# dgaddy/silent_speech

Hardware: AMD Instinct MI355X
Metric: EMG frames/s training (transduction_model.py) (higher is better)
Workload: dtype bf16

## Files before the change

include/silent_speech_hip.h:

```cpp
#ifndef SILENT_SPEECH_HIP_H
#define SILENT_SPEECH_HIP_H
#include <stdint.h>
#ifdef __cplusplus
extern "C" {
#endif

#define SS_F32 0
#define SS_BF16 1
#define SS_F32X3 3

const char* ss_last_error(void);
#define SS_ABI_VERSION 23
int ss_abi_version(void);
const char* ss_target_arch(void);

typedef struct ss_rowmap {
    int64_t base;
    int64_t batch_stride;
    int64_t row_stride;
    int32_t rows_per_batch;
} ss_rowmap;

typedef struct ss_gemm_epilogue {
    const float* bias;
    const void* gate;
    float gate_scale;
    float alpha;
// ... 114 lines not shown

int ss_emg_prepare(int dtype, const float* x_raw, void* out_padded, float* shifted_copy, int B, int T0, int Cin, int shift, void* stream);

int ss_loss_index_tables(const int64_t* utt_dev, int n_utt, int32_t* vo_pred, int32_t* vo_tgt, int32_t* si_tgt, int32_t* si_base,
                         int32_t* si_res, void* stream);
int ss_frame_lse(const float* head, int64_t ld, int col0, int ncls, int rows, float* lse, int32_t* argmax, void* stream);
int ss_voiced_loss(const float* head, int64_t ld, int n_mel, int n_phone, const float* lse, const int32_t* argmax, const float* Y,
                   const int64_t* phones, const int32_t* pred_row, const int32_t* tgt_row, int nframes, float lam, float inv_total,
                   float* dhead, float* loss_accum, int32_t* correct_accum, void* stream);
int ss_silent_cost_skewed(const float* head, int64_t ld, int n_mel, const float* lse, const float* Y, const int64_t* phones,
                          const int64_t* desc_dev, int n, int max_n, int max_m, float lam, void* workspace, int32_t* results, void* stream);
int ss_silent_loss(const float* head, int64_t ld, int n_mel, int n_phone, const float* lse, const int32_t* argmax, const float* Y,
                   const int64_t* phones, const int32_t* results, const int32_t* tgt_row, const int32_t* pred_base,
                   const int32_t* res_idx, int nframes, float lam, float inv_total, float* dhead, float* loss_accum,
                   int32_t* correct_accum, void* stream);
int ss_phoneme_confusion(const int32_t* argmax, const int64_t* phones, const int32_t* results, const int32_t* vo_pred, const int32_t* vo_tgt,
                         int n_voiced, const int32_t* si_tgt, const int32_t* si_base, const int32_t* si_res, int n_silent_frames,
                         int32_t* confusion, int n_phone, void* stream);

int ss_ctc_loss(const float* logits, int64_t ld, int V, int blank, const float* lse, const int64_t* desc_dev, int n_utt, int max_target_len,
                int64_t rows, const int32_t* targets, float* alpha_ws, float* beta_ws, float* nll, float* dlogits, float* loss, void* stream);

int64_t ss_ctc_beam_workspace_bytes(int n_utt, int64_t total_frames, int beam_width);
int ss_ctc_beam_search(const float* logits, int64_t ld, int V, int blank, int64_t rows, const float* lse, const int64_t* utt_dev, int n_utt,
                       int64_t total_frames, int beam_width, int n_best, const float* lm, float alpha, float beta, void* workspace, int max_len,
                       int32_t* labels, int32_t* lengths, float* scores, float* ctc_scores, void* stream);

typedef struct ss_word_lm {
    const int32_t* lex_child;
    const int32_t* lex_word;
// ... 184 lines not shown
```

silent_speech_amd/_lib.py:

```python
import ctypes
import os

import torch

_HERE = os.path.dirname(os.path.abspath(__file__))
_LIB_PATH = os.environ.get('SS_AMD_LIBRARY') or os.path.join(_HERE, 'lib', 'libsilent_speech_hip.so')

SS_F32, SS_BF16, SS_F64, SS_F32X3 = 0, 1, 2, 3
ABI_VERSION = 23
OP_KC, OP_OC = 0, 1


class RowMap(ctypes.Structure):
    _fields_ = [('base', ctypes.c_int64), ('batch_stride', ctypes.c_int64), ('row_stride', ctypes.c_int64),
                ('rows_per_batch', ctypes.c_int32)]


class GemmEpilogue(ctypes.Structure):
    _fields_ = [('bias', ctypes.c_void_p), ('gate', ctypes.c_void_p), ('gate_scale', ctypes.c_float),
                ('alpha', ctypes.c_float), ('relu', ctypes.c_int32), ('dropout_p', ctypes.c_float),
                ('seed', ctypes.c_uint64), ('rng_stream', ctypes.c_uint32), ('mode', ctypes.c_int32),
                ('col_mod', ctypes.c_int32), ('col_mul', ctypes.c_int32), ('col_div_mul', ctypes.c_int32),
                ('log_clamp', ctypes.c_float), ('c2', ctypes.c_void_p), ('cmap2', RowMap), ('col_stride2', ctypes.c_int64),
                ('col_sum', ctypes.c_void_p), ('col_sumsq', ctypes.c_void_p), ('col_shift', ctypes.c_void_p),
# ... 22 lines not shown
    _fields_ = [('lex_child', ctypes.c_void_p), ('lex_word', ctypes.c_void_p), ('uni_logp', ctypes.c_void_p), ('uni_bo', ctypes.c_void_p),
                ('bi_keys', ctypes.c_void_p), ('bi_logp', ctypes.c_void_p), ('bi_bo', ctypes.c_void_p), ('tri_keys', ctypes.c_void_p),
                ('tri_logp', ctypes.c_void_p), ('n_nodes', ctypes.c_int32), ('n_vocab', ctypes.c_int32), ('n_uni', ctypes.c_int32),
                ('start', ctypes.c_int32), ('bi_slots', ctypes.c_int32), ('bi_probe', ctypes.c_int32), ('tri_slots', ctypes.c_int32),
                ('tri_probe', ctypes.c_int32)]


class WordStateLm(ctypes.Structure):
    _fields_ = [('lex_child', ctypes.c_void_p), ('lex_word', ctypes.c_void_p), ('uni_logp', ctypes.c_void_p), ('st_bo', ctypes.c_void_p),
                ('st_shorter', ctypes.c_void_p), ('arc_keys', ctypes.c_void_p), ('arc_logp', ctypes.c_void_p), ('arc_next', ctypes.c_void_p),
                ('n_nodes', ctypes.c_int32), ('n_vocab', ctypes.c_int32), ('n_uni', ctypes.c_int32), ('n_states', ctypes.c_int32),
                ('start_state', ctypes.c_int32), ('arc_slots', ctypes.c_int32), ('arc_probe', ctypes.c_int32), ('order', ctypes.c_int32)]


_P, _I, _F, _L = ctypes.c_void_p, ctypes.c_int, ctypes.c_float, ctypes.c_int64
_U64, _U32 = ctypes.c_uint64, ctypes.c_uint32

SIGNATURES = {
    'ss_gemm': [_I, _I, _I, _I, _P, _P, _P, _I, _I, _I, ctypes.POINTER(RowMap), ctypes.POINTER(RowMap),
                ctypes.POINTER(RowMap), ctypes.POINTER(GemmEpilogue), _I, _P],
    'ss_gemm_dw_grouped': [_I, ctypes.POINTER(DwJob), _P],
    'ss_split_planes': [_P, _P, _P, _L, _P],
    'ss_gemm_planes': [_I, _P, _P, _P, _P, _P, _I, _I, _I, ctypes.POINTER(RowMap), ctypes.POINTER(RowMap), ctypes.POINTER(RowMap), ctypes.POINTER(GemmEpilogue), _P],
    'ss_permute3d': [_P, _I, _P, _I, _I, _I, _I, _L, _L, _L, _I, _I, _F, _I, _P],
    'ss_permute3d_batch': [_P, _P, _I, _I, _P],
    'ss_dtw_align': [_P, _P, _I, _I, _I, _P, _P, _P],
    'ss_dtw_align_skewed': [_P, _I, _P, _P, _P],
    'ss_reflect_pad_ragged': [_P, _P, _P, _P, _I, _I, _I, _L, _I, _P],
    'ss_concat_pad': [_P, _I, _P, _L, _I, _P],
    'ss_dtw_cumulative': [_I, _P, _L, _L, _I, _I, _P, _P, _P],
# ... 14 lines not shown
    'ss_bn_backward_sums': [_I, _P, _I, _P, _I, _P, _I, _P, _P, _P, _I, _P, _P, _P, _P, _P, _P, _P, _P, _I, _I, _I, _I, _P, _P, _P, _P, _P],
    'ss_bn_backward_apply': [_I, _P, _I, _P, _I, _P, _I, _P, _P, _P, _P, _I, _P, _P, _P, _P, ctypes.c_double, _P, _I, _P, _I, _I, _I, _I, _I, _P, _P, _P],
    'ss_colsum': [_I, _P, _I, _I, _L, _P, _P, _P],
    'ss_add_dropout_layernorm_forward': [_I, _P, _P, _P, _P, _P, _P, _P, _I, _I, _F, _F, _U64, _U32, _P],
    'ss_add_dropout_layernorm_forward_planes': [_I, _P, _P, _P, _P, _P, _P, _P, _P, _P, _I, _I, _F, _F, _U64, _U32, _P],
    'ss_layernorm_backward': [_I, _P, _P, _P, _P, _P, _P, _P, _P, _P, _I, _I, _F, _U64, _U32, _P],
    'ss_layernorm_backward_bias': [_I, _P, _P, _P, _P, _P, _P, _P, _P, _P, _P, _I, _I, _F, _U64, _U32, _P],
    'ss_layernorm_backward_ws': [_I, _P, _P, _P, _P, _P, _P, _P, _P, _P, _P, _P, _L, _I, _I, _F, _U64, _U32, _P],
    'ss_layernorm_backward_ws_planes': [_I, _P, _P, _P, _P, _P, _P, _P, _P, _P, _P, _P, _P, _P, _L, _I, _I, _F, _U64, _U32, _P],
    'ss_emg_prepare': [_I, _P, _P, _P, _I, _I, _I, _I, _P],
    'ss_frame_lse': [_P, _L, _I, _I, _I, _P, _P, _P],
    'ss_loss_index_tables': [_P, _I, _P, _P, _P, _P, _P, _P],
    'ss_voiced_loss': [_P, _L, _I, _I, _P, _P, _P, _P, _P, _P, _I, _F, _F, _P, _P, _P, _P],
    'ss_silent_cost_skewed': [_P, _L, _I, _P, _P, _P, _P, _I, _I, _I, _F, _P, _P, _P],
    'ss_silent_loss': [_P, _L, _I, _I, _P, _P, _P, _P, _P, _P, _P, _P, _I, _F, _F, _P, _P, _P, _P],
    'ss_phoneme_confusion': [_P, _P, _P, _P, _P, _I, _P, _P, _P, _I, _P, _I, _P],
    'ss_ctc_loss': [_P, _L, _I, _I, _P, _P, _I, _I, _L, _P, _P, _P, _P, _P, _P, _P],
    'ss_ctc_beam_search': [_P, _L, _I, _I, _L, _P, _P, _I, _L, _I, _I, _P, _F, _F, _P, _I, _P, _P, _P, _P, _P],
    'ss_ctc_word_beam_search': [_P, _L, _I, _I, _I, _L, _P, _P, _I, _L, _I, _I, ctypes.POINTER(WordLm), _F, _F, _P, _I, _P, _P, _P, _P, _P, _P],
    'ss_word_ngram_score': [ctypes.POINTER(WordLm), _P, _L, _P, _P],
    'ss_ctc_word_state_beam_search': [_P, _L, _I, _I, _I, _L, _P, _P, _I, _L, _I, _I, ctypes.POINTER(WordStateLm), _F, _F, _P, _I, _P, _P, _P, _P, _P, _P],
    'ss_word_state_score': [ctypes.POINTER(WordStateLm), _P, _L, _P, _P, _P],
    'ss_ctc_align': [_P, _L, _I, _I, _L, _P, _P, _I, _L, _I, _P, _L, _P, _P, _P, _P, _P, _P, _P],
    'ss_edit_distance': [_P, _L, _P, _L, _P, _L, _P, _P, _P, _P, _L, _P, _P],
    'ss_nbest_risk': [_P, _L, _P, _L, _P, _I, _I, _P, _P, _L, _P, _P, _P],
    'ss_ctc_nbest_logp': [_P, _L, _I, _I, _L, _P, _P, _I, _P, _L, _I, _P, _L, _P, _L, _P, _P],
    'ss_ctc_nbest_backward': [_P, _L, _I, _I, _L, _P, _P, _I, _L, _P, _P, _L, _P, _P, _P, _P],
    'ss_nbest_expected_risk': [_P, _P, _L, _P, _I, ctypes.c_double, _P, _P, _P, _P, _P],
    'ss_adamw_step': [_P, _P, _P, _P, _L, _F, _F, _F, _F, _F, _I, _F, _P],
    'ss_cast_f32': [_P, _P, _I, _L, _P],
# ... 162 lines not shown
```

silent_speech_amd/csrc/loss.hip:

```cpp
#include "common.h"
#include <stdlib.h>
#include "silent_speech_hip.h"
#include <math.h>

namespace {
constexpr int DESC = 10;
enum { D_N = 0, D_M, D_PRED_ROW0, D_TGT_ROW0, D_UNUSED, D_SK_OFF, D_DIRS_OFF, D_BND_OFF, D_RES_OFF };
constexpr int DW = 4, DR = 4;
__device__ __forceinline__ long long dtw_strips_d(long long n) { long long rows = n - 1, cap = DW * 64 * DR; return rows <= 0 ? 0 : (rows + cap - 1) / cap; }
__device__ __forceinline__ long long dtw_tsteps_d(long long m) { return m <= 1 ? 0 : (m - 1) + 63; }
}

__global__ void frame_lse_kernel(const float* __restrict__ head, long long ld, int col0, int ncls, int rows, float* __restrict__ lse, int* __restrict__ amax)
{
    const int lane = threadIdx.x & 63, wpb = blockDim.x >> 6;
    for (int r = blockIdx.x * wpb + (threadIdx.x >> 6); r < rows; r += gridDim.x * wpb) {
        const float* a = head + (long long)r * ld + col0;
        float mx = -INFINITY; int mi = 0x7fffffff;
        for (int c = lane; c < ncls; c += 64) { float v = a[c]; if (v > mx) { mx = v; mi = c; } }
        const float gmx = wave_max(mx);
        int cand = (mx == gmx) ? mi : 0x7fffffff;
#pragma unroll
        for (int m = 32; m >= 1; m >>= 1) { int o = __shfl_xor(cand, m); cand = o < cand ? o : cand; }
        float s = 0.f;
// ... 44 lines not shown
__device__ __forceinline__ void loss_block_commit(float lsum, int csum, float inv_total, float* loss_acc, int* correct_acc)
{
    __shared__ float ls[16];
    __shared__ int cs[16];
    const int lane = threadIdx.x & 63, w = threadIdx.x >> 6, wpb = blockDim.x >> 6;
    if (lane == 0) { ls[w] = lsum; cs[w] = csum; }
    __syncthreads();
    if (threadIdx.x == 0) {
        float a = 0.f; int c = 0;
        for (int i = 0; i < wpb; ++i) { a += ls[i]; c += cs[i]; }
        if (a != 0.f) atomicAdd(loss_acc, a * inv_total);
        if (c) atomicAdd(correct_acc, c);
    }
}

__global__ void voiced_loss_kernel(const float* __restrict__ head, long long ld, int n_mel, int n_ph, const float* __restrict__ lse, const int* __restrict__ amax,
                                   const float* __restrict__ Y, const long long* __restrict__ phones, const int* __restrict__ pred_row, const int* __restrict__ tgt_row,
                                   int nframes, float lam, float inv_total, float* __restrict__ dhead, float* __restrict__ loss_acc, int* __restrict__ correct_acc)
{
    const int lane = threadIdx.x & 63, wpb = blockDim.x >> 6;
    float lsum = 0.f; int csum = 0;
    for (int f = blockIdx.x * wpb + (threadIdx.x >> 6); f < nframes; f += gridDim.x * wpb) {
        const int pr = pred_row[f], tr = tgt_row[f];
        const float* p = head + (long long)pr * ld; const float* y = Y + (long long)tr * n_mel;
        float* dp = dhead + (long long)pr * ld;
        float ss = 0.f;
        for (int c = lane; c < n_mel; c += 64) { float d = y[c] - p[c] + 1e-6f; ss += d * d; }
        const float dist = sqrtf(wave_sum(ss));
        const float gs = dist > 0.f ? inv_total / dist : 0.f;
        for (int c = lane; c < n_mel; c += 64) dp[c] = -(y[c] - p[c] + 1e-6f) * gs;
        const int ph = (int)phones[tr];
        const float L = lse[pr];
        for (int c = lane; c < n_ph; c += 64) dp[n_mel + c] = lam * inv_total * (expf(p[n_mel + c] - L) - (c == ph ? 1.f : 0.f));
        if (lane == 0) { lsum += dist + lam * (L - p[n_mel + ph]); csum += amax[pr] == ph; }
    }
    loss_block_commit(lsum, csum, inv_total, loss_acc, correct_acc);
}

extern "C" int ss_voiced_loss(const float* head, int64_t ld, int n_mel, int n_phone, const float* lse, const int32_t* argmax, const float* Y, const int64_t* phones,
                              const int32_t* pred_row, const int32_t* tgt_row, int nframes, float lam, float inv_total,
                              float* dhead, float* loss_accum, int32_t* correct_accum, void* stream)
{
    SS_CHECK(nframes >= 0, "ss_voiced_loss: negative frame count");
    if (nframes == 0) return 0;
    SS_CHECK(head && lse && argmax && Y && phones && pred_row && tgt_row && dhead && loss_accum && correct_accum, "ss_voiced_loss: null pointer");
    int blocks = (nframes + 3) / 4; if (blocks > 1024) blocks = 1024;
    SS_LAUNCH(voiced_loss_kernel, dim3(blocks), dim3(256), 0, stream, head, (long long)ld, n_mel, n_phone, lse, (const int*)argmax, Y, (const long long*)phones,
              (const int*)pred_row, (const int*)tgt_row, nframes, lam, inv_total, dhead, loss_accum, (int*)correct_accum);
    SS_LAUNCH_CHECK("ss_voiced_loss");
    return 0;
}

constexpr int YMAX = 128;
__device__ __forceinline__ float quad_bcast(float v, int k) {
#if defined(SS_EMU)
    return __shfl(v, (int)((threadIdx.x & 63) & ~3) + k);
#else
    switch (k) {
    case 0: return __int_as_float(__builtin_amdgcn_update_dpp(0, __float_as_int(v), 0x00, 0xf, 0xf, true));
    case 1: return __int_as_float(__builtin_amdgcn_update_dpp(0, __float_as_int(v), 0x55, 0xf, 0xf, true));
    case 2: return __int_as_float(__builtin_amdgcn_update_dpp(0, __float_as_int(v), 0xAA, 0xf, 0xf, true));
    default: return __int_as_float(__builtin_amdgcn_update_dpp(0, __float_as_int(v), 0xFF, 0xf, 0xf, true));
    }
#endif
}
template <int NQ>
__device__ __forceinline__ float quad_shared_sqdist(const float* __restrict__ p, int r, const f32x4 (&yv)[YMAX / 4]) {
    f32x4 own[NQ];
#pragma unroll
    for (int q = 0; q < NQ; ++q) own[q] = *(const f32x4*)(p + (r * NQ + q) * 4);
    float ss = 0.f;
#pragma unroll
    for (int k = 0; k < 4; ++k) {
#pragma unroll
        for (int q = 0; q < NQ; ++q) {
            const f32x4 b = yv[k * NQ + q];
            const float a0 = quad_bcast(own[q][0], k), a1 = quad_bcast(own[q][1], k), a2 = quad_bcast(own[q][2], k), a3 = quad_bcast(own[q][3], k);
            const float d0 = a0 - b[0], d1 = a1 - b[1], d2 = a2 - b[2], d3 = a3 - b[3];
            ss += d0 * d0; ss += d1 * d1; ss += d2 * d2; ss += d3 * d3;
        }
    }
    return ss;
}

__global__ __launch_bounds__(256) void silent_cost_skewed_kernel(const float* __restrict__ head, long long ld, int n_mel, const float* __restrict__ lse, const float* __restrict__ Y,
                                                                 const long long* __restrict__ phones, const long long* __restrict__ desc, float lam, unsigned char* __restrict__ ws, int* __restrict__ results, int CT)
{
    const long long* d = desc + (long long)blockIdx.y * DESC;
    const int N = (int)d[D_N], M = (int)d[D_M];
    const long long p0 = d[D_PRED_ROW0], y0 = d[D_TGT_ROW0];
    int* res = results + d[D_RES_OFF];
    for (int i = blockIdx.x * blockDim.x + threadIdx.x; i < N; i += gridDim.x * blockDim.x) res[i] = 0;
    const long long ts = dtw_tsteps_d(M), nkw = dtw_strips_d(N) * DW;
    if (ts <= 0) return;
    const long long tchunks = (ts + CT - 1) / CT, nwork = nkw * tchunks;
    float* sk = (float*)(ws + d[D_SK_OFF]);
    const int l = threadIdx.x >> 2, r = threadIdx.x & 3;
    for (long long wk = blockIdx.x; wk < nwork; wk += gridDim.x) {
        const long long kw = wk / tchunks, t0 = (wk - kw * tchunks) * CT;
        const long long i = 1 + (kw * 64 + l) * DR + r;
        const bool iv = i < N;
        f32x4 yv[YMAX / 4];
        int ph = 0;
        if (iv) {
            const float* y = Y + (y0 + i) * n_mel;
#pragma unroll
            for (int q = 0; q < YMAX / 4; ++q) if (q * 4 < n_mel) yv[q] = *(const f32x4*)(y + q * 4);
            ph = (int)phones[y0 + i];
        }
        const long long tend = t0 + CT < ts ? t0 + CT : ts;
        if (n_mel == 80) {
            for (long long t = t0; t < tend; ++t) {
                const long long j = t + 1 - l;
                const bool jv = j >= 1 && j < M;
                const float* p = head + (p0 + (jv ? j : 1)) * ld;
                const float ss = quad_shared_sqdist<5>(p, r, yv);
                float c = INFINITY;
                if (jv && iv) c = sqrtf(ss) + lam * (lse[p0 + j] - p[n_mel + ph]);
                sk[((kw * ts + t) * 64 + l) * DR + r] = c;
            }
            continue;
        }
        for (long long t = t0; t < tend; ++t) {
            const long long j = t + 1 - l;
            float c = INFINITY;
            if (iv && j >= 1 && j < M) {
                const float* p = head + (p0 + j) * ld;
// ... 11 lines not shown
            sk[((kw * ts + t) * 64 + l) * DR + r] = c;
        }
    }
}

extern "C" int ss_silent_cost_skewed(const float* head, int64_t ld, int n_mel, const float* lse, const float* Y, const int64_t* phones,
                                     const int64_t* desc_dev, int n, int max_n, int max_m, float lam, void* workspace, int32_t* results, void* stream)
{
    SS_CHECK(n >= 0, "ss_silent_cost_skewed: negative batch");
    if (n == 0) return 0;
    SS_CHECK(head && lse && Y && phones && desc_dev && workspace && results, "ss_silent_cost_skewed: null pointer");
    SS_CHECK(n_mel % 4 == 0 && ld % 4 == 0, "ss_silent_cost_skewed: n_mel and ld must be multiples of 4 (16-byte rows)");
    SS_CHECK(n_mel <= YMAX, "ss_silent_cost_skewed: at most %d mel bins", YMAX);
    long long strips = max_n <= 1 ? 0 : (max_n - 1 + DW * 64 * DR - 1) / (DW * 64 * DR);
    const long long ts_max = max_m <= 1 ? 0 : max_m - 1 + 63;
    static const int CT = getenv("SS_COST_CT") ? atoi(getenv("SS_COST_CT")) : 16;
    long long blocks = strips * DW * ((ts_max + CT - 1) / CT);
    if (blocks < (max_n + 255) / 256) blocks = (max_n + 255) / 256;
    if (blocks > 4096) blocks = 4096;
    if (blocks < 1) blocks = 1;
    SS_LAUNCH(silent_cost_skewed_kernel, dim3((unsigned)blocks, n), dim3(256), 0, stream, head, (long long)ld, n_mel, lse, Y, (const long long*)phones,
              (const long long*)desc_dev, lam, (unsigned char*)workspace, (int*)results, CT);
    SS_LAUNCH_CHECK("ss_silent_cost_skewed");
    return 0;
}

__global__ void silent_loss_kernel(const float* __restrict__ head, long long ld, int n_mel, int n_ph, const float* __restrict__ lse, const int* __restrict__ amax,
                                   const float* __restrict__ Y, const long long* __restrict__ phones, const int* __restrict__ results,
                                   const int* __restrict__ tgt_row, const int* __restrict__ pred_base, const int* __restrict__ res_idx,
                                   int nframes, float lam, float inv_total, float* __restrict__ dhead, float* __restrict__ loss_acc, int* __restrict__ correct_acc)
{
    const int lane = threadIdx.x & 63, wpb = blockDim.x >> 6;
    float lsum = 0.f; int csum = 0;
    for (int f = blockIdx.x * wpb + (threadIdx.x >> 6); f < nframes; f += gridDim.x * wpb) {
        const int tr = tgt_row[f], pr = pred_base[f] + results[res_idx[f]];
        const float* p = head + (long long)pr * ld; const float* y = Y + (long long)tr * n_mel;
        float* dp = dhead + (long long)pr * ld;
        float ss = 0.f;
        for (int c = lane; c < n_mel; c += 64) { float d = p[c] - y[c]; ss += d * d; }
        const float dist = sqrtf(wave_sum(ss));
        const float gs = dist > 0.f ? inv_total / dist : 0.f;
        for (int c = lane; c < n_mel; c += 64) atomicAdd(dp + c, (p[c] - y[c]) * gs);
        const int ph = (int)phones[tr];
        const float L = lse[pr];
        for (int c = lane; c < n_ph; c += 64) atomicAdd(dp + n_mel + c, lam * inv_total * (expf(p[n_mel + c] - L) - (c == ph ? 1.f : 0.f)));
        if (lane == 0) { lsum += dist + lam * (L - p[n_mel + ph]); csum += amax[pr] == ph; }
    }
    loss_block_commit(lsum, csum, inv_total, loss_acc, correct_acc);
}

extern "C" int ss_silent_loss(const float* head, int64_t ld, int n_mel, int n_phone, const float* lse, const int32_t* argmax, const float* Y, const int64_t* phones,
                              const int32_t* results, const int32_t* tgt_row, const int32_t* pred_base, const int32_t* res_idx, int nframes,
                              float lam, float inv_total, float* dhead, float* loss_accum, int32_t* correct_accum, void* stream)
{
    SS_CHECK(nframes >= 0, "ss_silent_loss: negative frame count");
    if (nframes == 0) return 0;
    SS_CHECK(head && lse && argmax && Y && phones && results && tgt_row && pred_base && res_idx && dhead && loss_accum && correct_accum, "ss_silent_loss: null pointer");
    int blocks = (nframes + 3) / 4; if (blocks > 1024) blocks = 1024;
    SS_LAUNCH(silent_loss_kernel, dim3(blocks), dim3(256), 0, stream, head, (long long)ld, n_mel, n_phone, lse, (const int*)argmax, Y, (const long long*)phones,
              (const int*)results, (const int*)tgt_row, (const int*)pred_base, (const int*)res_idx, nframes, lam, inv_total, dhead, loss_accum, (int*)correct_accum);
    SS_LAUNCH_CHECK("ss_silent_loss");
    return 0;
}

__global__ void phoneme_confusion_kernel(const int* __restrict__ amax, const long long* __restrict__ phones, const int* __restrict__ results,
                                         const int* __restrict__ vo_pred, const int* __restrict__ vo_tgt, int n_voiced,
                                         const int* __restrict__ si_tgt, const int* __restrict__ si_base, const int* __restrict__ si_res, int n_silent,
                                         int* __restrict__ conf, int n_phone)
{
    for (int i = blockIdx.x * blockDim.x + threadIdx.x; i < n_voiced + n_silent; i += gridDim.x * blockDim.x) {
        int p, t;
        if (i < n_voiced) { p = amax[vo_pred[i]]; t = (int)phones[vo_tgt[i]]; }
        else { const int k = i - n_voiced; p = amax[si_base[k] + results[si_res[k]]]; t = (int)phones[si_tgt[k]]; }
        if ((unsigned)p < (unsigned)n_phone && (unsigned)t < (unsigned)n_phone) atomicAdd(conf + p * n_phone + t, 1);
        else atomicAdd(conf + n_phone * n_phone, 1);
    }
// ... 18 lines not shown
```

silent_speech_amd/ops.py:

```python
import ctypes

import torch

from . import _lib
from ._lib import OP_KC, OP_OC, RowMap, GemmEpilogue


def rowmap(row_stride, rows_per_batch=0, batch_stride=0, base=0):
    return RowMap(int(base), int(batch_stride), int(row_stride), int(rows_per_batch))


PROFILER = None


class LaunchProfiler(object):

    def __init__(self):
        self.records = []
        self.enabled = True

    def run(self, name, flops, nbytes, fn):
        if not self.enabled or not torch.cuda.is_available():
            return fn()
        s = torch.cuda.Event(enable_timing=True)
# ... 9 lines not shown
        agg = {}
        for name, flops, nbytes, s, e in self.records:
            a = agg.setdefault(name, dict(calls=0, flops=0.0, bytes=0.0, seconds=0.0))
            a['calls'] += 1
            a['flops'] += flops
            a['bytes'] += nbytes
            a['seconds'] += s.elapsed_time(e) * 1e-3
        self.records = []
        return agg


def timed(name, flops, nbytes, fn):
    if PROFILER is not None:
        return PROFILER.run(name, flops, nbytes, fn)
    return fn()


def gemm(A, B, C, M, N, K, amap, bmap, cmap, **kw):
    return _gemm_full(A, B, C, M, N, K, amap, bmap, cmap, {}, **kw)


def permute3d(inp, out, dims, strides, valid1=None, valid2=None, scale=1.0, accumulate=False):
    d0, d1, d2 = dims
    assert out.numel() >= d0 * d1 * d2 and out.is_contiguous()
    rc = _lib.lib().ss_permute3d(_lib.ptr(inp), _lib.dtype_code(inp.dtype), _lib.ptr(out), _lib.dtype_code(out.dtype),
                                 d0, d1, d2, strides[0], strides[1], strides[2],
                                 d1 if valid1 is None else valid1, d2 if valid2 is None else valid2,
                                 float(scale), int(accumulate), _lib.stream_of(out))
    _lib.check(rc, 'ss_permute3d')
    return out
# ... 438 lines not shown
```

silent_speech_amd/torch_ops.py:

```python
import ctypes
import weakref
from typing import Optional, Tuple

import torch
from torch import Tensor

from . import _lib, ops

_L = _lib.lib
_p = _lib.ptr

_models = {}
_next_id = [1]
_KEEP = 2


def model_handle(model):
    h = getattr(model, '_op_handle', None)
    if h is None:
        h = model._op_handle = _next_id[0]
        _next_id[0] += 1
        _models[h] = weakref.ref(model)
        model._saved_ctx = {}
    return h
# ... 66 lines not shown


@model_forward_ragged.register_fake
def _(x_raw, lens, handle):
    m = _model(handle)
    n_head_cols = (m.num_outs + (m.num_aux_outs or 0) + 7) // 8 * 8
    return x_raw.new_empty((x_raw.shape[0] * (x_raw.shape[1] // 8), n_head_cols), dtype=torch.float32)


@torch.library.custom_op('silent_speech::dtw_loss', mutates_args=())
def dtw_loss(head: Tensor, Y: Tensor, phones: Tensor, idx: Tensor, desc: Tensor, n_mel: int, n_ph: int, lam: float, inv_total: float,
             n_voiced: int, n_silent_frames: int, n_silent: int, ws_bytes: int, res_total: int, max_n: int, max_m: int,
             cells: float, perimeter: float) -> Tuple[Tensor, Tensor, Tensor, Tensor, Tensor]:
    dev = head.device
    M, ld = head.shape
    st = _lib.stream_of(head)
    nv, ns = max(n_voiced, 1), max(n_silent_frames, 1)
    vo_pred, vo_tgt = idx[:nv], idx[nv:2 * nv]
    si_tgt, si_base, si_res = idx[2 * nv:2 * nv + ns], idx[2 * nv + ns:2 * nv + 2 * ns], idx[2 * nv + 2 * ns:]
    lse = torch.empty(M, dtype=torch.float32, device=dev)
    amax = torch.empty(M, dtype=torch.int32, device=dev)
    dhead = torch.zeros_like(head)
    loss = torch.zeros(1, dtype=torch.float32, device=dev)
    correct = torch.zeros(1, dtype=torch.int32, device=dev)
    _lib.check(_L().ss_frame_lse(_p(head), ld, n_mel, n_ph, M, _p(lse), _p(amax), st), 'ss_frame_lse')
    if n_voiced:
        _lib.check(_L().ss_voiced_loss(_p(head), ld, n_mel, n_ph, _p(lse), _p(amax), _p(Y), _p(phones), _p(vo_pred), _p(vo_tgt),
                                       n_voiced, lam, inv_total, _p(dhead), _p(loss), _p(correct), st), 'ss_voiced_loss')
    results = torch.empty(max(res_total, 1), dtype=torch.int32, device=dev)
    if n_silent:
        ws = torch.empty(max(ws_bytes, 256), dtype=torch.uint8, device=dev)
        ops.timed('silent_cost_skewed_kernel', 0, 4.0 * cells + 4.0 * (n_mel + n_ph) * perimeter,
                  lambda: _lib.check(_L().ss_silent_cost_skewed(_p(head), ld, n_mel, _p(lse), _p(Y), _p(phones), _p(desc), n_silent, max_n, max_m,
                                                                lam, _p(ws), _p(results), st), 'ss_silent_cost_skewed'))
        ops.timed('dtw_kernel', 0, 8.0 * cells,
                  lambda: _lib.check(_L().ss_dtw_align_skewed(_p(desc), n_silent, _p(ws), _p(results), st), 'ss_dtw_align_skewed'))
        _lib.check(_L().ss_silent_loss(_p(head), ld, n_mel, n_ph, _p(lse), _p(amax), _p(Y), _p(phones), _p(results), _p(si_tgt),
                                       _p(si_base), _p(si_res), n_silent_frames, lam, inv_total, _p(dhead), _p(loss), _p(correct), st), 'ss_silent_loss')
    return loss, correct, dhead, results, amax


@dtw_loss.register_fake
def _(head, Y, phones, idx, desc, n_mel, n_ph, lam, inv_total, n_voiced, n_silent_frames, n_silent, ws_bytes, res_total, max_n, max_m, cells, perimeter):
    M = head.shape[0]
    return (head.new_empty(1), head.new_empty(1, dtype=torch.int32), torch.empty_like(head), head.new_empty(max(res_total, 1), dtype=torch.int32),
            head.new_empty(M, dtype=torch.int32))


def _dtw_setup(ctx, inputs, output):
    ctx.save_for_backward(output[2])


def _dtw_bwd(ctx, g_loss, g_correct, g_dhead, g_results, g_amax):
# ... 793 lines not shown
```

Baseline: 1.683 million.

## Fuse DTW loss forward into one host call with side-stream overlap

Moves the whole DTW loss forward sequence into a single C entry point. The voiced loss kernel now runs on a forked side stream alongside the silent cost/DTW chain, and per-block partial sums replace atomics, reduced by a final finish kernel. The separate torch zero-fills are replaced by one async memset. The silent cost kernel for 80 mel bins is also templated to process U=4 time steps per iteration. This cuts Python launch overhead and serialization, at the cost of extra stream/event management and more complex code.

```diff
diff --git a/include/silent_speech_hip.h b/include/silent_speech_hip.h
--- a/include/silent_speech_hip.h
+++ b/include/silent_speech_hip.h
@@ -10,7 +10,7 @@
 #define SS_F32X3 3
 
 const char* ss_last_error(void);
-#define SS_ABI_VERSION 23
+#define SS_ABI_VERSION 24
 int ss_abi_version(void);
 const char* ss_target_arch(void);
 
@@ -155,6 +155,14 @@
                    const int64_t* phones, const int32_t* results, const int32_t* tgt_row, const int32_t* pred_base,
                    const int32_t* res_idx, int nframes, float lam, float inv_total, float* dhead, float* loss_accum,
                    int32_t* correct_accum, void* stream);
+typedef void (*ss_launch_hook)(const char* kernel, int begin, void* arg);
+int ss_dtw_loss_scratch_bytes(void);
+int ss_dtw_loss_forward(const float* head, int64_t ld, int rows, int n_mel, int n_phone, const float* Y, const int64_t* phones,
+                        const int32_t* vo_pred, const int32_t* vo_tgt, int n_voiced,
+                        const int32_t* si_tgt, const int32_t* si_base, const int32_t* si_res, int n_silent_frames,
+                        const int64_t* desc_dev, int n_silent, int max_n, int max_m, float lam, float inv_total,
+                        float* lse, int32_t* argmax, float* dhead, void* scratch, void* workspace, int32_t* results,
+                        float* loss, int32_t* correct, ss_launch_hook hook, void* hook_arg, void* stream);
 int ss_phoneme_confusion(const int32_t* argmax, const int64_t* phones, const int32_t* results, const int32_t* vo_pred, const int32_t* vo_tgt,
                          int n_voiced, const int32_t* si_tgt, const int32_t* si_base, const int32_t* si_res, int n_silent_frames,
                          int32_t* confusion, int n_phone, void* stream);
diff --git a/silent_speech_amd/_lib.py b/silent_speech_amd/_lib.py
--- a/silent_speech_amd/_lib.py
+++ b/silent_speech_amd/_lib.py
@@ -7,7 +7,7 @@
 _LIB_PATH = os.environ.get('SS_AMD_LIBRARY') or os.path.join(_HERE, 'lib', 'libsilent_speech_hip.so')
 
 SS_F32, SS_BF16, SS_F64, SS_F32X3 = 0, 1, 2, 3
-ABI_VERSION = 23
+ABI_VERSION = 24
 OP_KC, OP_OC = 0, 1
 
 
@@ -60,6 +60,7 @@
 
 
 _P, _I, _F, _L = ctypes.c_void_p, ctypes.c_int, ctypes.c_float, ctypes.c_int64
+LAUNCH_HOOK = ctypes.CFUNCTYPE(None, ctypes.c_char_p, ctypes.c_int, ctypes.c_void_p)
 _U64, _U32 = ctypes.c_uint64, ctypes.c_uint32
 
 SIGNATURES = {
@@ -104,6 +105,8 @@
     'ss_voiced_loss': [_P, _L, _I, _I, _P, _P, _P, _P, _P, _P, _I, _F, _F, _P, _P, _P, _P],
     'ss_silent_cost_skewed': [_P, _L, _I, _P, _P, _P, _P, _I, _I, _I, _F, _P, _P, _P],
     'ss_silent_loss': [_P, _L, _I, _I, _P, _P, _P, _P, _P, _P, _P, _P, _I, _F, _F, _P, _P, _P, _P],
+    'ss_dtw_loss_forward': [_P, _L, _I, _I, _I, _P, _P, _P, _P, _I, _P, _P, _P, _I, _P, _I, _I, _I, _F, _F, _P, _P, _P, _P, _P, _P, _P, _P, LAUNCH_HOOK, _P, _P],
+    'ss_dtw_loss_scratch_bytes': [],
     'ss_phoneme_confusion': [_P, _P, _P, _P, _P, _I, _P, _P, _P, _I, _P, _I, _P],
     'ss_ctc_loss': [_P, _L, _I, _I, _P, _P, _I, _I, _L, _P, _P, _P, _P, _P, _P, _P],
     'ss_ctc_beam_search': [_P, _L, _I, _I, _L, _P, _P, _I, _L, _I, _I, _P, _F, _F, _P, _I, _P, _P, _P, _P, _P],
diff --git a/silent_speech_amd/csrc/loss.hip b/silent_speech_amd/csrc/loss.hip
--- a/silent_speech_amd/csrc/loss.hip
+++ b/silent_speech_amd/csrc/loss.hip
@@ -2,6 +2,7 @@
 #include <stdlib.h>
 #include "silent_speech_hip.h"
 #include <math.h>
+#include <mutex>
 
 namespace {
 constexpr int DESC = 10;
@@ -82,9 +83,44 @@
     }
 }
 
+__device__ __forceinline__ void loss_block_store(float lsum, int csum, float inv_total, float* loss_part, int* correct_part)
+{
+    __shared__ float ls[16];
+    __shared__ int cs[16];
+    const int lane = threadIdx.x & 63, w = threadIdx.x >> 6, wpb = blockDim.x >> 6;
+    if (lane == 0) { ls[w] = lsum; cs[w] = csum; }
+    __syncthreads();
+    if (threadIdx.x == 0) {
+        float a = 0.f; int c = 0;
+        for (int i = 0; i < wpb; ++i) { a += ls[i]; c += cs[i]; }
+        loss_part[blockIdx.x] = a * inv_total; correct_part[blockIdx.x] = c;
+    }
+}
+__device__ __forceinline__ void loss_block_end(float lsum, int csum, float inv_total, float* loss_acc, int* correct_acc, float* loss_part, int* correct_part)
+{
+    if (loss_part) loss_block_store(lsum, csum, inv_total, loss_part, correct_part);
+    else loss_block_commit(lsum, csum, inv_total, loss_acc, correct_acc);
+}
+constexpr int LOSS_MAX_BLOCKS = 1024;
+inline int loss_blocks(int nframes) { int b = (nframes + 3) / 4; return b > LOSS_MAX_BLOCKS ? LOSS_MAX_BLOCKS : b; }
+
+__global__ void loss_finish_kernel(const float* __restrict__ lv, const int* __restrict__ cv, int nv, const float* __restrict__ lsil, const int* __restrict__ csil, int nsil,
+                                   float* __restrict__ loss, int* __restrict__ correct)
+{
+    const int lane = threadIdx.x;
+    float v = 0.f, s = 0.f; int c = 0;
+    for (int i = lane; i < nv; i += 64) { v += lv[i]; c += cv[i]; }
+    for (int i = lane; i < nsil; i += 64) { s += lsil[i]; c += csil[i]; }
+    v = wave_sum(v); s = wave_sum(s);
+#pragma unroll
+    for (int m = 32; m >= 1; m >>= 1) c += __shfl_xor(c, m);
+    if (lane == 0) { loss[0] = v + s; correct[0] = c; }
+}
+
 __global__ void voiced_loss_kernel(const float* __restrict__ head, long long ld, int n_mel, int n_ph, const float* __restrict__ lse, const int* __restrict__ amax,
                                    const float* __restrict__ Y, const long long* __restrict__ phones, const int* __restrict__ pred_row, const int* __restrict__ tgt_row,
-                                   int nframes, float lam, float inv_total, float* __restrict__ dhead, float* __restrict__ loss_acc, int* __restrict__ correct_acc)
+                                   int nframes, float lam, float inv_total, float* __restrict__ dhead, float* __restrict__ loss_acc, int* __restrict__ correct_acc,
+                                   float* __restrict__ loss_part, int* __restrict__ correct_part)
 {
     const int lane = threadIdx.x & 63, wpb = blockDim.x >> 6;
     float lsum = 0.f; int csum = 0;
@@ -102,7 +138,17 @@
         for (int c = lane; c < n_ph; c += 64) dp[n_mel + c] = lam * inv_total * (expf(p[n_mel + c] - L) - (c == ph ? 1.f : 0.f));
         if (lane == 0) { lsum += dist + lam * (L - p[n_mel + ph]); csum += amax[pr] == ph; }
     }
-    loss_block_commit(lsum, csum, inv_total, loss_acc, correct_acc);
+    loss_block_end(lsum, csum, inv_total, loss_acc, correct_acc, loss_part, correct_part);
+}
+
+static int voiced_loss_launch(const float* head, int64_t ld, int n_mel, int n_phone, const float* lse, const int32_t* argmax, const float* Y, const int64_t* phones,
+                              const int32_t* pred_row, const int32_t* tgt_row, int nframes, float lam, float inv_total,
+                              float* dhead, float* loss_accum, int32_t* correct_accum, float* loss_part, int32_t* correct_part, void* stream)
+{
+    SS_LAUNCH(voiced_loss_kernel, dim3(loss_blocks(nframes)), dim3(256), 0, stream, head, (long long)ld, n_mel, n_phone, lse, (const int*)argmax, Y, (const long long*)phones,
+              (const int*)pred_row, (const int*)tgt_row, nframes, lam, inv_total, dhead, loss_accum, (int*)correct_accum, loss_part, (int*)correct_part);
+    SS_LAUNCH_CHECK("ss_voiced_loss");
+    return 0;
 }
 
 extern "C" int ss_voiced_loss(const float* head, int64_t ld, int n_mel, int n_phone, const float* lse, const int32_t* argmax, const float* Y, const int64_t* phones,
@@ -112,14 +158,12 @@
     SS_CHECK(nframes >= 0, "ss_voiced_loss: negative frame count");
     if (nframes == 0) return 0;
     SS_CHECK(head && lse && argmax && Y && phones && pred_row && tgt_row && dhead && loss_accum && correct_accum, "ss_voiced_loss: null pointer");
-    int blocks = (nframes + 3) / 4; if (blocks > 1024) blocks = 1024;
-    SS_LAUNCH(voiced_loss_kernel, dim3(blocks), dim3(256), 0, stream, head, (long long)ld, n_mel, n_phone, lse, (const int*)argmax, Y, (const long long*)phones,
-              (const int*)pred_row, (const int*)tgt_row, nframes, lam, inv_total, dhead, loss_accum, (int*)correct_accum);
-    SS_LAUNCH_CHECK("ss_voiced_loss");
-    return 0;
+    return voiced_loss_launch(head, ld, n_mel, n_phone, lse, argmax, Y, phones, pred_row, tgt_row, nframes, lam, inv_total, dhead, loss_accum, correct_accum,
+                              nullptr, nullptr, stream);
 }
 
 constexpr int YMAX = 128;
+constexpr int SS_COST_CT_DEFAULT = 16;
 __device__ __forceinline__ float quad_bcast(float v, int k) {
 #if defined(SS_EMU)
     return __shfl(v, (int)((threadIdx.x & 63) & ~3) + k);
@@ -150,7 +194,76 @@
     }
     return ss;
 }
-
+template <int TERM>
+__device__ __forceinline__ float sq_acc80(float ss, float d) {
+#if defined(SS_EMU)
+    return ss + d * d;
+#else
+    if constexpr (TERM < 70) return __builtin_fmaf(d, d, ss);
+    else {
+#pragma clang fp contract(off)
+        const float sq = d * d;
+        return ss + sq;
+    }
+#endif
+}
+__device__ __forceinline__ void reg_pin(float& v) {
+#if !defined(SS_EMU)
+    asm volatile("" : "+v"(v));
+#endif
+}
+template <int U, int K, int Q>
+__device__ __forceinline__ void sqdist80_piece(const f32x4 (&own)[U][5], const f32x4 (&yv)[YMAX / 4], float (&ss)[U]) {
+    const f32x4 b = yv[K * 5 + Q];
+#pragma unroll
+    for (int u = 0; u < U; ++u) {
+        const float a0 = quad_bcast(own[u][Q][0], K), a1 = quad_bcast(own[u][Q][1], K), a2 = quad_bcast(own[u][Q][2], K), a3 = quad_bcast(own[u][Q][3], K);
+        const float d0 = a0 - b[0], d1 = a1 - b[1], d2 = a2 - b[2], d3 = a3 - b[3];
+        constexpr int T = (K * 5 + Q) * 4;
+        ss[u] = sq_acc80<T>(ss[u], d0); ss[u] = sq_acc80<T + 1>(ss[u], d1); ss[u] = sq_acc80<T + 2>(ss[u], d2); ss[u] = sq_acc80<T + 3>(ss[u], d3);
+    }
+#pragma unroll
+    for (int u = 0; u < U; ++u) reg_pin(ss[u]);
+    sched_fence();
+}
+template <int U, int K>
+__device__ __forceinline__ void sqdist80_lane(const f32x4 (&own)[U][5], const f32x4 (&yv)[YMAX / 4], float (&ss)[U]) {
+    sqdist80_piece<U, K, 0>(own, yv, ss); sqdist80_piece<U, K, 1>(own, yv, ss); sqdist80_piece<U, K, 2>(own, yv, ss);
+    sqdist80_piece<U, K, 3>(own, yv, ss); sqdist80_piece<U, K, 4>(own, yv, ss);
+}
+template <int U>
+__device__ __forceinline__ void quad_shared_sqdist80_multi(const float* const (&p)[U], int r, const f32x4 (&yv)[YMAX / 4], float (&ss)[U]) {
+    f32x4 own[U][5];
+#pragma unroll
+    for (int u = 0; u < U; ++u) {
+#pragma unroll
+        for (int q = 0; q < 5; ++q) own[u][q] = *(const f32x4*)(p[u] + (r * 5 + q) * 4);
+    }
+#pragma unroll
+    for (int u = 0; u < U; ++u) ss[u] = 0.f;
+    sqdist80_lane<U, 0>(own, yv, ss); sqdist80_lane<U, 1>(own, yv, ss); sqdist80_lane<U, 2>(own, yv, ss); sqdist80_lane<U, 3>(own, yv, ss);
+}
+template <int U>
+__device__ __forceinline__ void cost_cells80(const float* __restrict__ head, long long ld, const float* __restrict__ lse, long long p0, int M, int l, int r, bool iv, int ph,
+                                             float lam, const f32x4 (&yv)[YMAX / 4], long long t, float* __restrict__ skt)
+{
+    const float* p[U]; bool jv[U]; float ss[U];
+#pragma unroll
+    for (int u = 0; u < U; ++u) {
+        const long long j = t + u + 1 - l;
+        jv[u] = j >= 1 && j < M;
+        p[u] = head + (p0 + (jv[u] ? j : 1)) * ld;
+    }
+    quad_shared_sqdist80_multi<U>(p, r, yv, ss);
+#pragma unroll
+    for (int u = 0; u < U; ++u) {
+        float c = INFINITY;
+        if (jv[u] && iv) c = sqrtf(ss[u]) + lam * (lse[p0 + (t + u + 1 - l)] - p[u][80 + ph]);
+        skt[(long long)u * 64 * DR] = c;
+    }
+}
+
+template <bool MEL80, int U>
 __global__ __launch_bounds__(256) void silent_cost_skewed_kernel(const float* __restrict__ head, long long ld, int n_mel, const float* __restrict__ lse, const float* __restrict__ Y,
                                                                  const long long* __restrict__ phones, const long long* __restrict__ desc, float lam, unsigned char* __restrict__ ws, int* __restrict__ results, int CT)
 {
@@ -173,12 +286,16 @@
         if (iv) {
             const float* y = Y + (y0 + i) * n_mel;
 #pragma unroll
-            for (int q = 0; q < YMAX / 4; ++q) if (q * 4 < n_mel) yv[q] = *(const f32x4*)(y + q * 4);
+            for (int q = 0; q < (MEL80 ? 20 : YMAX / 4); ++q) if (MEL80 || q * 4 < n_mel) yv[q] = *(const f32x4*)(y + q * 4);
             ph = (int)phones[y0 + i];
         }
         const long long tend = t0 + CT < ts ? t0 + CT : ts;
-        if (n_mel == 80) {
-            for (long long t = t0; t < tend; ++t) {
+        if constexpr (MEL80) {
+            long long t = t0;
+            if constexpr (U > 1) {
+                for (; t + U <= tend; t += U) cost_cells80<U>(head, ld, lse, p0, M, l, r, iv, ph, lam, yv, t, sk + ((kw * ts + t) * 64 + l) * DR + r);
+                for (; t < tend; ++t) cost_cells80<1>(head, ld, lse, p0, M, l, r, iv, ph, lam, yv, t, sk + ((kw * ts + t) * 64 + l) * DR + r);
+            } else for (; t < tend; ++t) {
                 const long long j = t + 1 - l;
                 const bool jv = j >= 1 && j < M;
                 const float* p = head + (p0 + (jv ? j : 1)) * ld;
@@ -220,13 +337,20 @@
     SS_CHECK(n_mel <= YMAX, "ss_silent_cost_skewed: at most %d mel bins", YMAX);
     long long strips = max_n <= 1 ? 0 : (max_n - 1 + DW * 64 * DR - 1) / (DW * 64 * DR);
     const long long ts_max = max_m <= 1 ? 0 : max_m - 1 + 63;
-    static const int CT = getenv("SS_COST_CT") ? atoi(getenv("SS_COST_CT")) : 16;
+    const char* e_ct = getenv("SS_COST_CT"); const char* e_u = getenv("SS_COST_U");
+    const int CT = e_ct ? atoi(e_ct) : SS_COST_CT_DEFAULT, U = e_u ? atoi(e_u) : 4;
+    SS_CHECK(CT >= 1 && (U == 1 || U == 2 || U == 4), "ss_silent_cost_skewed: SS_COST_CT must be >= 1 and SS_COST_U one of 1, 2, 4");
     long long blocks = strips * DW * ((ts_max + CT - 1) / CT);
     if (blocks < (max_n + 255) / 256) blocks = (max_n + 255) / 256;
     if (blocks > 4096) blocks = 4096;
     if (blocks < 1) blocks = 1;
-    SS_LAUNCH(silent_cost_skewed_kernel, dim3((unsigned)blocks, n), dim3(256), 0, stream, head, (long long)ld, n_mel, lse, Y, (const long long*)phones,
-              (const long long*)desc_dev, lam, (unsigned char*)workspace, (int*)results, CT);
+#define SS_COST_LAUNCH(MEL80, U_) SS_LAUNCH(SS_KERNEL(silent_cost_skewed_kernel<MEL80, U_>), dim3((unsigned)blocks, n), dim3(256), 0, stream, head, (long long)ld, n_mel, lse, Y, \
+        (const long long*)phones, (const long long*)desc_dev, lam, (unsigned char*)workspace, (int*)results, CT)
+    if (n_mel != 80) SS_COST_LAUNCH(false, 1);
+    else if (U == 4) SS_COST_LAUNCH(true, 4);
+    else if (U == 2) SS_COST_LAUNCH(true, 2);
+    else SS_COST_LAUNCH(true, 1);
+#undef SS_COST_LAUNCH
     SS_LAUNCH_CHECK("ss_silent_cost_skewed");
     return 0;
 }
@@ -234,7 +358,8 @@
 __global__ void silent_loss_kernel(const float* __restrict__ head, long long ld, int n_mel, int n_ph, const float* __restrict__ lse, const int* __restrict__ amax,
                                    const float* __restrict__ Y, const long long* __restrict__ phones, const int* __restrict__ results,
                                    const int* __restrict__ tgt_row, const int* __restrict__ pred_base, const int* __restrict__ res_idx,
-                                   int nframes, float lam, float inv_total, float* __restrict__ dhead, float* __restrict__ loss_acc, int* __restrict__ correct_acc)
+                                   int nframes, float lam, float inv_total, float* __restrict__ dhead, float* __restrict__ loss_acc, int* __restrict__ correct_acc,
+                                   float* __restrict__ loss_part, int* __restrict__ correct_part)
 {
     const int lane = threadIdx.x & 63, wpb = blockDim.x >> 6;
     float lsum = 0.f; int csum = 0;
@@ -252,7 +377,18 @@
         for (int c = lane; c < n_ph; c += 64) atomicAdd(dp + n_mel + c, lam * inv_total * (expf(p[n_mel + c] - L) - (c == ph ? 1.f : 0.f)));
         if (lane == 0) { lsum += dist + lam * (L - p[n_mel + ph]); csum += amax[pr] == ph; }
     }
-    loss_block_commit(lsum, csum, inv_total, loss_acc, correct_acc);
+    loss_block_end(lsum, csum, inv_total, loss_acc, correct_acc, loss_part, correct_part);
+}
+
+static int silent_loss_launch(const float* head, int64_t ld, int n_mel, int n_phone, const float* lse, const int32_t* argmax, const float* Y, const int64_t* phones,
+                              const int32_t* results, const int32_t* tgt_row, const int32_t* pred_base, const int32_t* res_idx, int nframes,
+                              float lam, float inv_total, float* dhead, float* loss_accum, int32_t* correct_accum, float* loss_part, int32_t* correct_part, void* stream)
+{
+    SS_LAUNCH(silent_loss_kernel, dim3(loss_blocks(nframes)), dim3(256), 0, stream, head, (long long)ld, n_mel, n_phone, lse, (const int*)argmax, Y, (const long long*)phones,
+              (const int*)results, (const int*)tgt_row, (const int*)pred_base, (const int*)res_idx, nframes, lam, inv_total, dhead, loss_accum, (int*)correct_accum,
+              loss_part, (int*)correct_part);
+    SS_LAUNCH_CHECK("ss_silent_loss");
+    return 0;
 }
 
 extern "C" int ss_silent_loss(const float* head, int64_t ld, int n_mel, int n_phone, const float* lse, const int32_t* argmax, const float* Y, const int64_t* phones,
@@ -262,10 +398,90 @@
     SS_CHECK(nframes >= 0, "ss_silent_loss: negative frame count");
     if (nframes == 0) return 0;
     SS_CHECK(head && lse && argmax && Y && phones && results && tgt_row && pred_base && res_idx && dhead && loss_accum && correct_accum, "ss_silent_loss: null pointer");
-    int blocks = (nframes + 3) / 4; if (blocks > 1024) blocks = 1024;
-    SS_LAUNCH(silent_loss_kernel, dim3(blocks), dim3(256), 0, stream, head, (long long)ld, n_mel, n_phone, lse, (const int*)argmax, Y, (const long long*)phones,
-              (const int*)results, (const int*)tgt_row, (const int*)pred_base, (const int*)res_idx, nframes, lam, inv_total, dhead, loss_accum, (int*)correct_accum);
-    SS_LAUNCH_CHECK("ss_silent_loss");
+    return silent_loss_launch(head, ld, n_mel, n_phone, lse, argmax, Y, phones, results, tgt_row, pred_base, res_idx, nframes, lam, inv_total, dhead, loss_accum, correct_accum,
+                              nullptr, nullptr, stream);
+}
+
+namespace {
+struct LossFork {
+    void* side = nullptr; bool ready = false;
+#if !defined(SS_EMU)
+    hipEvent_t ev_fork = 0, ev_join = 0;
+#endif
+};
+constexpr int LOSS_MAX_DEVICES = 64;
+LossFork* loss_fork_state()
+{
+#if defined(SS_EMU)
+    return nullptr;
+#else
+    static LossFork forks[LOSS_MAX_DEVICES];
+    static std::mutex mu;
+    std::lock_guard<std::mutex> lock(mu);
+    int dev = 0;
+    if (hipGetDevice(&dev) != hipSuccess || dev < 0 || dev >= LOSS_MAX_DEVICES) return nullptr;
+    LossFork& f = forks[dev];
+    if (!f.ready) {
+        hipStream_t s = nullptr;
+        if (hipStreamCreateWithFlags(&s, hipStreamNonBlocking) != hipSuccess) return nullptr;
+        if (hipEventCreateWithFlags(&f.ev_fork, hipEventDisableTiming) != hipSuccess || hipEventCreateWithFlags(&f.ev_join, hipEventDisableTiming) != hipSuccess) {
+            (void)hipStreamDestroy(s);
+            return nullptr;
+        }
+        f.side = s; f.ready = true;
+    }
+    return &f;
+#endif
+}
+}
+
+extern "C" int ss_dtw_loss_scratch_bytes(void) { return 4 * LOSS_MAX_BLOCKS * 4; }
+
+extern "C" int ss_dtw_loss_forward(const float* head, int64_t ld, int rows, int n_mel, int n_phone, const float* Y, const int64_t* phones,
+                                   const int32_t* vo_pred, const int32_t* vo_tgt, int n_voiced,
+                                   const int32_t* si_tgt, const int32_t* si_base, const int32_t* si_res, int n_silent_frames,
+                                   const int64_t* desc_dev, int n_silent, int max_n, int max_m, float lam, float inv_total,
+                                   float* lse, int32_t* argmax, float* dhead, void* scratch, void* workspace, int32_t* results,
+                                   float* loss, int32_t* correct, ss_launch_hook hook, void* hook_arg, void* stream)
+{
+    SS_CHECK(rows >= 0 && n_voiced >= 0 && n_silent >= 0 && n_silent_frames >= 0, "ss_dtw_loss_forward: negative count");
+    SS_CHECK(head && lse && argmax && dhead && scratch && loss && correct, "ss_dtw_loss_forward: null pointer");
+    SS_CHECK(n_voiced == 0 || (Y && phones && vo_pred && vo_tgt), "ss_dtw_loss_forward: voiced tables missing");
+    SS_CHECK(n_silent == 0 || (Y && phones && si_tgt && si_base && si_res && desc_dev && workspace && results), "ss_dtw_loss_forward: silent tables missing");
+    SS_CHECK(ss_memset_async(dhead, 0, (size_t)rows * (size_t)ld * sizeof(float), stream), "ss_dtw_loss_forward: memset failed");
+    if (ss_frame_lse(head, ld, n_mel, n_phone, rows, lse, argmax, stream)) return 1;
+    float* lv = (float*)scratch; int32_t* cv = (int32_t*)scratch + LOSS_MAX_BLOCKS;
+    float* lsil = (float*)scratch + 2 * LOSS_MAX_BLOCKS; int32_t* csil = (int32_t*)scratch + 3 * LOSS_MAX_BLOCKS;
+    LossFork* fk = (n_voiced && n_silent && !hook) ? loss_fork_state() : nullptr;
+    void* vstream = stream;
+#if !defined(SS_EMU)
+    if (fk) {
+        SS_CHECK(hipEventRecord(fk->ev_fork, (hipStream_t)stream) == hipSuccess && hipStreamWaitEvent((hipStream_t)fk->side, fk->ev_fork, 0) == hipSuccess,
+                 "ss_dtw_loss_forward: fork failed");
+        vstream = fk->side;
+    }
+#endif
+    int rc = 0;
+    if (n_voiced) rc = voiced_loss_launch(head, ld, n_mel, n_phone, lse, argmax, Y, phones, vo_pred, vo_tgt, n_voiced, lam, inv_total, dhead, nullptr, nullptr, lv, cv, vstream);
+    if (!rc && n_silent) {
+        if (hook) hook("silent_cost_skewed_kernel", 1, hook_arg);
+        rc = ss_silent_cost_skewed(head, ld, n_mel, lse, Y, phones, desc_dev, n_silent, max_n, max_m, lam, workspace, results, stream);
+        if (hook) { hook("silent_cost_skewed_kernel", 0, hook_arg); hook("dtw_kernel", 1, hook_arg); }
+        if (!rc) rc = ss_dtw_align_skewed(desc_dev, n_silent, workspace, results, stream);
+        if (hook) hook("dtw_kernel", 0, hook_arg);
+        if (!rc && n_silent_frames) rc = silent_loss_launch(head, ld, n_mel, n_phone, lse, argmax, Y, phones, results, si_tgt, si_base, si_res, n_silent_frames, lam, inv_total,
+                                                             dhead, nullptr, nullptr, lsil, csil, stream);
+    }
+#if !defined(SS_EMU)
+    if (fk && (hipEventRecord(fk->ev_join, (hipStream_t)fk->side) != hipSuccess || hipStreamWaitEvent((hipStream_t)stream, fk->ev_join, 0) != hipSuccess) && !rc) {
+        ss_set_error("ss_dtw_loss_forward: join failed");
+        rc = 1;
+    }
+#endif
+    if (rc) return rc;
+    SS_LAUNCH(loss_finish_kernel, dim3(1), dim3(64), 0, stream, (const float*)lv, (const int*)cv, n_voiced ? loss_blocks(n_voiced) : 0,
+              (const float*)lsil, (const int*)csil, (n_silent && n_silent_frames) ? loss_blocks(n_silent_frames) : 0, loss, (int*)correct);
+    SS_LAUNCH_CHECK("ss_dtw_loss_forward");
     return 0;
 }
 
diff --git a/silent_speech_amd/ops.py b/silent_speech_amd/ops.py
--- a/silent_speech_amd/ops.py
+++ b/silent_speech_amd/ops.py
@@ -47,6 +47,23 @@
     if PROFILER is not None:
         return PROFILER.run(name, flops, nbytes, fn)
     return fn()
+
+
+def launch_hook(rows):
+    prof = PROFILER
+    if prof is None or not prof.enabled or not torch.cuda.is_available():
+        return _lib.LAUNCH_HOOK()
+    started = {}
+
+    def hook(name, begin, _arg):
+        ev = torch.cuda.Event(enable_timing=True)
+        ev.record()
+        if begin:
+            started[name] = ev
+        else:
+            flops, nbytes = rows[name.decode()]
+            prof.records.append((name.decode(), float(flops), float(nbytes), started.pop(name), ev))
+    return _lib.LAUNCH_HOOK(hook)
 
 
 def gemm(A, B, C, M, N, K, amap, bmap, cmap, **kw):
diff --git a/silent_speech_amd/torch_ops.py b/silent_speech_amd/torch_ops.py
--- a/silent_speech_amd/torch_ops.py
+++ b/silent_speech_amd/torch_ops.py
@@ -104,29 +104,23 @@
              cells: float, perimeter: float) -> Tuple[Tensor, Tensor, Tensor, Tensor, Tensor]:
     dev = head.device
     M, ld = head.shape
-    st = _lib.stream_of(head)
     nv, ns = max(n_voiced, 1), max(n_silent_frames, 1)
     vo_pred, vo_tgt = idx[:nv], idx[nv:2 * nv]
     si_tgt, si_base, si_res = idx[2 * nv:2 * nv + ns], idx[2 * nv + ns:2 * nv + 2 * ns], idx[2 * nv + 2 * ns:]
     lse = torch.empty(M, dtype=torch.float32, device=dev)
     amax = torch.empty(M, dtype=torch.int32, device=dev)
-    dhead = torch.zeros_like(head)
-    loss = torch.zeros(1, dtype=torch.float32, device=dev)
-    correct = torch.zeros(1, dtype=torch.int32, device=dev)
-    _lib.check(_L().ss_frame_lse(_p(head), ld, n_mel, n_ph, M, _p(lse), _p(amax), st), 'ss_frame_lse')
-    if n_voiced:
-        _lib.check(_L().ss_voiced_loss(_p(head), ld, n_mel, n_ph, _p(lse), _p(amax), _p(Y), _p(phones), _p(vo_pred), _p(vo_tgt),
-                                       n_voiced, lam, inv_total, _p(dhead), _p(loss), _p(correct), st), 'ss_voiced_loss')
+    dhead = torch.empty_like(head)
+    loss = torch.empty(1, dtype=torch.float32, device=dev)
+    correct = torch.empty(1, dtype=torch.int32, device=dev)
+    scratch = torch.empty(_L().ss_dtw_loss_scratch_bytes(), dtype=torch.uint8, device=dev)
     results = torch.empty(max(res_total, 1), dtype=torch.int32, device=dev)
-    if n_silent:
-        ws = torch.empty(max(ws_bytes, 256), dtype=torch.uint8, device=dev)
-        ops.timed('silent_cost_skewed_kernel', 0, 4.0 * cells + 4.0 * (n_mel + n_ph) * perimeter,
-                  lambda: _lib.check(_L().ss_silent_cost_skewed(_p(head), ld, n_mel, _p(lse), _p(Y), _p(phones), _p(desc), n_silent, max_n, max_m,
-                                                                lam, _p(ws), _p(results), st), 'ss_silent_cost_skewed'))
-        ops.timed('dtw_kernel', 0, 8.0 * cells,
-                  lambda: _lib.check(_L().ss_dtw_align_skewed(_p(desc), n_silent, _p(ws), _p(results), st), 'ss_dtw_align_skewed'))
-        _lib.check(_L().ss_silent_loss(_p(head), ld, n_mel, n_ph, _p(lse), _p(amax), _p(Y), _p(phones), _p(results), _p(si_tgt),
-                                       _p(si_base), _p(si_res), n_silent_frames, lam, inv_total, _p(dhead), _p(loss), _p(correct), st), 'ss_silent_loss')
+    ws = torch.empty(max(ws_bytes, 256), dtype=torch.uint8, device=dev) if n_silent else None
+    hook = ops.launch_hook({'silent_cost_skewed_kernel': (0, 4.0 * cells + 4.0 * (n_mel + n_ph) * perimeter),
+                            'dtw_kernel': (0, 8.0 * cells)})
+    _lib.check(_L().ss_dtw_loss_forward(_p(head), ld, M, n_mel, n_ph, _p(Y), _p(phones), _p(vo_pred), _p(vo_tgt), n_voiced,
+                                        _p(si_tgt), _p(si_base), _p(si_res), n_silent_frames, _p(desc), n_silent, max_n, max_m, lam, inv_total,
+                                        _p(lse), _p(amax), _p(dhead), _p(scratch), _p(ws), _p(results), _p(loss), _p(correct),
+                                        hook, None, _lib.stream_of(head)), 'ss_dtw_loss_forward')
     return loss, correct, dhead, results, amax
 
 
```

After: 1.681 million. About the same (-0.2%).
